# Tongji-MIC-Lab/TDVC

Hardware: AMD Instinct MI355X
Metric: 1080p P-frames/sec (encode + reconstruct, lambda=2048 config) (higher is better)
Workload: dtype f16; 1 GPU; 1x 1920x1080 (padded 1088x1920) 7-frame synthetic GOP (seed 1234), batch 1, P-frames coded in GOP order; gop=7, batch=1, parallelism=gop-sharded x1, weights=closed-form filler (no checkpoint ships)

## Files before the change

tdvc_amd/csrc/conv_mfma.hip:

```cpp
#include "conv_common.h"

using convk::ConvParams;

namespace {

constexpr int TH = 8, TW = 32;

template <int CK8, int MT, int STRIDE, bool LEAN = false>
__global__ __launch_bounds__(256, LEAN ? 3 : 1) void conv_mfma_kernel(const ConvParams p) {
  extern __shared__ __attribute__((aligned(16))) unsigned char smem[];
  constexpr int CK = CK8 * 8;
  constexpr int PS = (CK8 == 1) ? 16 : CK * 2 + 16;
  int* tapoff = reinterpret_cast<int*>(smem);
  unsigned char* tile = smem + 256;

  const int tid = threadIdx.x, lane = tid & 63, wave = tid >> 6;
  const int hh = lane >> 5, r = lane & 31;
  const int tile_id = p.reverse ? (int)gridDim.x - 1 - tdvc_xcd_tile(blockIdx.x) : tdvc_xcd_tile(blockIdx.x);
  const int tx = tile_id % p.tiles_x, ty = tile_id / p.tiles_x;
  const int cb = blockIdx.y, n = blockIdx.z;

  const int TIH = (TH - 1) * STRIDE + p.kh;
  const int TIW = (TW - 1) * STRIDE + p.kw;
  const int HALFW = (TIW + 1) >> 1;
  const int TIWp = (STRIDE == 2) ? 2 * HALFW : TIW;

  if (tid < p.ntaps) {
    const int dy = p.tap_dy[tid], dx = p.tap_dx[tid];
    tapoff[tid] = (STRIDE == 2) ? (dy * TIWp + (dx & 1) * HALFW + (dx >> 1)) * PS : (dy * TIWp + dx) * PS;
  }

  int base[2];
#pragma unroll
  for (int nt = 0; nt < 2; ++nt) base[nt] = (((wave * 2 + nt) * STRIDE) * TIWp + r) * PS;

  f32x16 acc[MT][2];
#pragma unroll
  for (int mt = 0; mt < MT; ++mt)
#pragma unroll
    for (int nt = 0; nt < 2; ++nt)
#pragma unroll
      for (int i = 0; i < 16; ++i) acc[mt][nt][i] = 0.f;

  const half_t* xn = p.x + (long)n * p.x_sn;
  const int iy0 = ty * TH * STRIDE - p.pad, ix0 = tx * TW * STRIDE - p.pad;
  const int total = TIH * TIW * CK8;

  for (int ch = 0; ch < p.nchunks; ++ch) {
    if (ch > 0) __syncthreads();
    for (int idx = tid; idx < total; idx += 256) {
      const int c8 = idx % CK8;
      const int pix = idx / CK8;
      const int c = pix % TIW, rr = pix / TIW;
      const int iy = iy0 + rr, ix = ix0 + c;
      const int cg = ch * CK + c8 * 8;
      half8 v = {0, 0, 0, 0, 0, 0, 0, 0};
      if (iy >= 0 && iy < p.H && ix >= 0 && ix < p.W && cg < p.Cin)
        v = *reinterpret_cast<const half8*>(xn + ((long)iy * p.W + ix) * p.x_sp + cg);
      if (p.square) v = v * v;
      const int cpos = (STRIDE == 2) ? ((c & 1) * HALFW + (c >> 1)) : c;
      *reinterpret_cast<half8*>(tile + (rr * TIWp + cpos) * PS + c8 * 16) = v;
    }
    __syncthreads();

    const half_t* wp[MT];
#pragma unroll
    for (int mt = 0; mt < MT; ++mt)
      wp[mt] = p.w + ((((long)(cb * MT + mt) * p.nchunks + ch) * p.steps) * 64 + lane) * 8;

    if constexpr (CK8 == 1) {
      for (int s = 0; s < p.steps; ++s) {
        int tap = 2 * s + hh;
        tap = tap < p.ntaps ? tap : p.ntaps - 1;
        const int toff = tapoff[tap];
        half8 a[MT], b[2];
#pragma unroll
        for (int mt = 0; mt < MT; ++mt) { a[mt] = *reinterpret_cast<const half8*>(wp[mt]); wp[mt] += 512; }
#pragma unroll
        for (int nt = 0; nt < 2; ++nt) b[nt] = *reinterpret_cast<const half8*>(tile + base[nt] + toff);
#pragma unroll
        for (int mt = 0; mt < MT; ++mt)
#pragma unroll
          for (int nt = 0; nt < 2; ++nt)
            acc[mt][nt] = __builtin_amdgcn_mfma_f32_32x32x16_f16(a[mt], b[nt], acc[mt][nt], 0, 0, 0);
      }
    } else {
      for (int tap = 0; tap < p.ntaps; ++tap) {
        const int toff = tapoff[tap] + hh * 16;
#pragma unroll
        for (int s2 = 0; s2 < CK8 / 2; ++s2) {
          half8 a[MT], b[2];
#pragma unroll
          for (int mt = 0; mt < MT; ++mt) { a[mt] = *reinterpret_cast<const half8*>(wp[mt]); wp[mt] += 512; }
#pragma unroll
          for (int nt = 0; nt < 2; ++nt)
            b[nt] = *reinterpret_cast<const half8*>(tile + base[nt] + toff + s2 * 32);
#pragma unroll
          for (int mt = 0; mt < MT; ++mt)
#pragma unroll
            for (int nt = 0; nt < 2; ++nt)
              acc[mt][nt] = __builtin_amdgcn_mfma_f32_32x32x16_f16(a[mt], b[nt], acc[mt][nt], 0, 0, 0);
        }
      }
    }
  }

  if constexpr (MT == 2 && LEAN) {
    __syncthreads();
    convk::epilogue_simple_rows<2, false, 2>(p, acc, p.bias + cb * 64, tile + wave * (32 * 144), n, cb * 64,
                                             ty * TH + wave * 2, tx * TW, lane, false);
    return;
  } else if constexpr (MT == 2) {
    if (p.simple) {
      __syncthreads();
      convk::epilogue_simple_rows<2, false, 1>(p, acc, p.bias + cb * 64, tile + wave * (32 * 144), n, cb * 64,
                                               ty * TH + wave * 2, tx * TW, lane, false);
      return;
    }
  }
  const int ox = tx * TW + r;
#pragma unroll
  for (int nt = 0; nt < 2; ++nt) {
    const int oy = ty * TH + wave * 2 + nt;
    if (oy >= p.Ho || ox >= p.Wo) continue;
#pragma unroll
    for (int mt = 0; mt < MT; ++mt) {
#pragma unroll
      for (int g = 0; g < 4; ++g) {
        const int co = (cb * MT + mt) * 32 + 8 * g + 4 * hh;
        float v[4];
#pragma unroll
        for (int i = 0; i < 4; ++i) v[i] = acc[mt][nt][4 * g + i];
        convk::epilogue4(p, n, oy, ox, co, v);
      }
    }
  }
}

template <int CK8, int MT, int STRIDE>
int launch(const ConvParams& p, dim3 grid, size_t lds, hipStream_t st) {
  if constexpr (MT == 2) {
    if (p.simple == 2) {
      hipLaunchKernelGGL((conv_mfma_kernel<CK8, MT, STRIDE, true>), grid, dim3(256), lds, st, p);
      return tdvc_launch_status("tdvc_conv2d");
    }
  }
  hipLaunchKernelGGL((conv_mfma_kernel<CK8, MT, STRIDE, false>), grid, dim3(256), lds, st, p);
  return tdvc_launch_status("tdvc_conv2d");
}

template <int CK8, int MT>
int launch_s(const ConvParams& p, int stride, dim3 grid, size_t lds, hipStream_t st) {
  return stride == 1 ? launch<CK8, MT, 1>(p, grid, lds, st) : launch<CK8, MT, 2>(p, grid, lds, st);
}

template <int CK8>
int launch_m(const ConvParams& p, int mt, int stride, dim3 grid, size_t lds, hipStream_t st) {
  return mt == 1 ? launch_s<CK8, 1>(p, stride, grid, lds, st) : launch_s<CK8, 2>(p, stride, grid, lds, st);
}

inline int lds_bytes(int ck, int kh, int kw, int stride) {
  const int ps = (ck == 8) ? 16 : ck * 2 + 16;
  const int tih = (TH - 1) * stride + kh, tiw = (TW - 1) * stride + kw;
  const int tiwp = stride == 2 ? 2 * ((tiw + 1) >> 1) : tiw;
  return 256 + tih * tiwp * ps;
}

inline int cout_tiles(int cout) { return cout <= 32 ? 1 : 2 * ((cout + 63) / 64); }

}

extern "C" int tdvc_conv_plan(int cin, int kh, int kw, int stride) {
  if (cin <= 0 || (cin % 8) != 0 || kh < 1 || kw < 1 || kh > 7 || kw > 7 || (stride != 1 && stride != 2)) {
    tdvc_set_error("tdvc_conv_plan: unsupported geometry cin=%d k=%dx%d stride=%d", cin, kh, kw, stride);
    return TDVC_EINVAL;
  }
  const int cands[4] = {64, 32, 16, 8};
  for (int i = 0; i < 4; ++i) {
    const int ck = cands[i];
    if (ck > cin && ck != 8) {
      if (cin % ck != 0 && cin < ck) continue;
    }
    if (lds_bytes(ck, kh, kw, stride) <= 64 * 1024) return ck;
  }
  tdvc_set_error("tdvc_conv_plan: no LDS plan for k=%dx%d stride=%d", kh, kw, stride);
  return TDVC_EINVAL;
}

extern "C" int64_t tdvc_conv_packed_bytes(int cout, int cin, int ntaps, int ck) {
  if (cout <= 0 || cin <= 0 || ntaps <= 0 || ntaps > TDVC_MAX_TAPS || (ck != 8 && ck != 16 && ck != 32 && ck != 64)) return TDVC_EINVAL;
  const int ck8 = ck / 8;
  const int64_t nchunks = (cin + ck - 1) / ck;
  const int64_t steps = (ntaps * ck8 + 1) / 2;
  return (int64_t)cout_tiles(cout) * nchunks * steps * 64 * 8 * 2;
}

extern "C" int tdvc_pack_conv_weights(const float* w, int cout, int cin_real, int cin, int kh, int kw,
                                      int ntaps, const int8_t* tap_dy, const int8_t* tap_dx, int ck, uint16_t* dst) {
  TDVC_CHECK(w && dst && tap_dy && tap_dx, "tdvc_pack_conv_weights: null pointer");
  TDVC_CHECK(tdvc_conv_packed_bytes(cout, cin, ntaps, ck) > 0, "tdvc_pack_conv_weights: bad geometry");
  TDVC_CHECK(cin_real <= cin, "tdvc_pack_conv_weights: cin_real > cin");
  const int ck8 = ck / 8;
  const int nchunks = (cin + ck - 1) / ck;
  const int steps = (ntaps * ck8 + 1) / 2;
  const int tiles = cout_tiles(cout);
  half_t* out = reinterpret_cast<half_t*>(dst);
  for (int t = 0; t < tiles; ++t)
    for (int ch = 0; ch < nchunks; ++ch)
      for (int s = 0; s < steps; ++s)
        for (int lane = 0; lane < 64; ++lane) {
          const int r = lane & 31, h = lane >> 5;
          const int co = t * 32 + r;
          const int kc = 2 * s + h;
          half_t* o = out + ((((int64_t)t * nchunks + ch) * steps + s) * 64 + lane) * 8;
          for (int j = 0; j < 8; ++j) {
            float v = 0.f;
            if (kc < ntaps * ck8 && co < cout) {
              const int tap = kc / ck8, c8 = kc % ck8;
              const int ci = ch * ck + c8 * 8 + j;
              const int dy = tap_dy[tap], dx = tap_dx[tap];
              if (ci < cin_real && dy >= 0 && dy < kh && dx >= 0 && dx < kw)
                v = w[(((int64_t)co * cin_real + ci) * kh + dy) * kw + dx];
            }
            o[j] = (half_t)v;
          }
        }
  return TDVC_OK;
}

int conv_direct_lds_bytes(const tdvc_conv_desc* d) { return lds_bytes(d->ck, d->kh, d->kw, d->stride); }
int conv_cout_tiles(int cout) { return cout_tiles(cout); }

int launch_conv_direct(const ConvParams& p, int ck8, int stride, int N, hipStream_t st) {
  const int tiles = cout_tiles(p.cout), mt = tiles == 1 ? 1 : 2;
  const int lds = lds_bytes(ck8 * 8, p.kh, p.kw, stride);
  const dim3 grid(p.tiles_x * ((p.Ho + TH - 1) / TH), tiles / mt, N);
  const size_t lds_v1 = (p.simple && lds < 256 + 4 * 32 * 144) ? 256 + 4 * 32 * 144 : lds;
  switch (ck8) {
    case 1: return launch_m<1>(p, mt, stride, grid, lds_v1, st);
    case 2: return launch_m<2>(p, mt, stride, grid, lds_v1, st);
    case 4: return launch_m<4>(p, mt, stride, grid, lds_v1, st);
    default: return launch_m<8>(p, mt, stride, grid, lds_v1, st);
  }
}
```

tdvc_amd/csrc/conv_n16.hip:

```cpp
#include "conv_common.h"

using convk::ConvParams;

namespace {

constexpr int N16_TH = 8, N16_TW = 64, N16_NTHR = 512;

struct N16Extra {
  int ksteps;
  int ps;
  int a_bytes;
  int ntiles, tiles_x;
  int cin_shift;
};

template <int NCB>
__global__ __launch_bounds__(N16_NTHR, 1) void conv_n16_kernel(const ConvParams p, const N16Extra e) {
  extern __shared__ __attribute__((aligned(16))) unsigned char smem[];
  unsigned char* wl = smem;
  unsigned char* tile = wl + e.a_bytes;
  const int tid = threadIdx.x, lane = tid & 63;
  const int wave = __builtin_amdgcn_readfirstlane(tid >> 6);
  const int px = lane & 15, kg = lane >> 4;
  const int TIW = N16_TW + p.kw - 1, TIH = N16_TH + p.kh - 1;
  const int cin = p.Cin, c8n = cin >> 3;

  for (int i = tid; i < e.ksteps * NCB * 64; i += N16_NTHR) {
    const int ln = i & 63, cb = (i >> 6) % NCB, S = (i >> 6) / NCB;
    const int q = 4 * S + (ln >> 4), s = q >> 1, h = q & 1;
    half8 v = {0, 0, 0, 0, 0, 0, 0, 0};
    if (s < p.steps) v = *reinterpret_cast<const half8*>(p.w + ((long)s * 64 + (16 * cb + (ln & 15)) + 32 * h) * 8);
    *reinterpret_cast<half8*>(wl + (long)i * 16) = v;
  }

  const int base = (wave * TIW + px) * e.ps;
  const int cstep = 16 * e.ps;
  auto frag_off = [&](int S) {
    const int kk0 = 32 * S + 8 * kg;
    const int tap = min(kk0 >> e.cin_shift, p.ntaps - 1);
    const int dy = tap / p.kw, dx = tap - dy * p.kw;
    return base + (dy * TIW + dx) * e.ps + (kk0 & (cin - 1)) * 2;
  };

  for (int tile_i = blockIdx.x; tile_i < e.ntiles; tile_i += gridDim.x) {
    const int per_img = e.tiles_x * ((p.Ho + N16_TH - 1) / N16_TH);
    const int n = tile_i / per_img, rem = tile_i - n * per_img;
    const int ty = rem / e.tiles_x, tx = rem - ty * e.tiles_x;
    const half_t* xn = p.x + (long)n * p.x_sn;
    const int iy0 = ty * N16_TH - p.pad, ix0 = tx * N16_TW - p.pad;
    __syncthreads();
    const int total = TIH * TIW * c8n;
    for (int idx0 = tid; idx0 < total; idx0 += 8 * N16_NTHR) {
      half8 v[8];
#pragma unroll
      for (int u = 0; u < 8; ++u) {
        const int idx = idx0 + u * N16_NTHR;
        const int pix = idx >> (e.cin_shift - 3), c8 = idx & (c8n - 1);
        const int rr = pix / TIW, cc = pix - rr * TIW;
        const int iy = iy0 + rr, ix = ix0 + cc;
        const bool ok = (int)(idx < total) & (int)(iy >= 0) & (int)(iy < p.H) & (int)(ix >= 0) & (int)(ix < p.W);
        const half_t* src = xn + ((long)(ok ? iy : 0) * p.W + (ok ? ix : 0)) * p.x_sp + c8 * 8;
        typedef unsigned u32x4 __attribute__((ext_vector_type(4)));
        u32x4 bits = *reinterpret_cast<const u32x4*>(src);
        unsigned m = ok ? 0xFFFFFFFFu : 0u;
        asm volatile("" : "+v"(m));
        bits &= m;
        v[u] = __builtin_bit_cast(half8, bits);
      }
#pragma unroll
      for (int u = 0; u < 8; ++u) {
        const int idx = idx0 + u * N16_NTHR;
        if (idx < total) {
          const int pix = idx >> (e.cin_shift - 3), c8 = idx & (c8n - 1);
          *reinterpret_cast<half8*>(tile + pix * e.ps + c8 * 16) = v[u];
        }
      }
    }
    __syncthreads();

    f32x4 acc[NCB][4];
#pragma unroll
    for (int cb = 0; cb < NCB; ++cb)
#pragma unroll
      for (int c = 0; c < 4; ++c) acc[cb][c] = f32x4{0.f, 0.f, 0.f, 0.f};

    half8 a0[NCB], b0[4], a1[NCB], b1[4];
    auto load = [&](int S, half8 (&a)[NCB], half8 (&b)[4]) {
      const int off = frag_off(S);
#pragma unroll
      for (int cb = 0; cb < NCB; ++cb) a[cb] = *reinterpret_cast<const half8*>(wl + ((S * NCB + cb) * 64 + lane) * 16);
#pragma unroll
      for (int c = 0; c < 4; ++c) b[c] = *reinterpret_cast<const half8*>(tile + off + c * cstep);
    };
    auto mm = [&](half8 (&a)[NCB], half8 (&b)[4]) {
#pragma unroll
      for (int c = 0; c < 4; ++c)
#pragma unroll
        for (int cb = 0; cb < NCB; ++cb) acc[cb][c] = __builtin_amdgcn_mfma_f32_16x16x32_f16(a[cb], b[c], acc[cb][c], 0, 0, 0);
    };
    const int KS = e.ksteps;
    load(0, a0, b0);
    for (int S = 0; S < KS; S += 2) {
      load(min(S + 1, KS - 1), a1, b1);
      mm(a0, b0);
      load(min(S + 2, KS - 1), a0, b0);
      if (S + 1 < KS) mm(a1, b1);
    }

    const int oy = ty * N16_TH + wave;
#pragma unroll
    for (int c = 0; c < 4; ++c) {
      const int ox = tx * N16_TW + 16 * c + px;
      if (oy < p.Ho && ox < p.Wo) {
#pragma unroll
        for (int cb = 0; cb < NCB; ++cb) {
          float v[4] = {acc[cb][c][0], acc[cb][c][1], acc[cb][c][2], acc[cb][c][3]};
          convk::epilogue4(p, n, oy, ox, 16 * cb + 4 * kg, v);
        }
      }
    }
  }
}

inline int n16_ps(int cin) { return 2 * cin + 16; }
inline int n16_ksteps(int ntaps, int cin) { return (ntaps * cin + 31) / 32; }
inline int n16_lds(int cin, int kh, int kw, int ntaps, int ncb) {
  return n16_ksteps(ntaps, cin) * ncb * 1024 + (N16_TH + kh - 1) * (N16_TW + kw - 1) * n16_ps(cin);
}

}

bool conv_n16_eligible(const tdvc_conv_desc* d, int Ho, int Wo) {
  const int cin = d->x.C;
  const bool cin_ok = cin == 8 || cin == 16 || cin == 32 || cin == 64;
  const bool dense = convk::taps_dense(d, d->kh, d->kw, d->pad);
  return cin_ok && dense && d->ck == cin && d->stride == 1 && d->cout <= 32 && !d->s2d && !d->square_input && !d->gdn &&
         (long)Ho * Wo >= convk::LARGE_MAP_PIXELS &&
         n16_lds(cin, d->kh, d->kw, d->ntaps, d->cout <= 16 ? 1 : 2) <= 150 * 1024;
}

int launch_conv_n16(const ConvParams& p, int N, hipStream_t st) {
  const int ncb = p.cout <= 16 ? 1 : 2;
  N16Extra e;
  e.ksteps = n16_ksteps(p.ntaps, p.Cin);
  e.ps = n16_ps(p.Cin);
  e.a_bytes = e.ksteps * ncb * 1024;
  e.tiles_x = (p.Wo + N16_TW - 1) / N16_TW;
  e.ntiles = N * e.tiles_x * ((p.Ho + N16_TH - 1) / N16_TH);
  e.cin_shift = p.Cin == 8 ? 3 : p.Cin == 16 ? 4 : p.Cin == 32 ? 5 : 6;
  const int lds = n16_lds(p.Cin, p.kh, p.kw, p.ntaps, ncb);
  const int per_cu = lds <= 78 * 1024 ? 2 : 1;
  int grid = e.ntiles < 256 * per_cu ? e.ntiles : 256 * per_cu;
  const auto go = ncb == 1 ? convk::launch_big_lds<&conv_n16_kernel<1>, ConvParams, N16Extra> : convk::launch_big_lds<&conv_n16_kernel<2>, ConvParams, N16Extra>;
  return go("tdvc_conv2d(n16)", 160 * 1024, dim3(grid), dim3(N16_NTHR), lds, st, p, e);
}
```

Before: 47.65 frames/s.

## Add wide-tile MFMA conv kernel and prefetch pipeline for n16 conv

Adds a new direct-conv kernel for single-cout-tile stride-1 layers on large maps. It uses 16-row tiles with 32x32x16 MFMAs over four row tiles per wave and a double-buffered LDS ring for weights. Separately, the n16 kernel gains a register prefetch of the next tile's input, overlapping global loads with MFMA compute, plus a precomputed LDS table of k-step offsets and a three-stage fragment pipeline. Both are on by default through debug toggles, at the cost of more registers, more LDS, and more template variants.

```diff
diff --git a/tdvc_amd/csrc/conv_mfma.hip b/tdvc_amd/csrc/conv_mfma.hip
--- a/tdvc_amd/csrc/conv_mfma.hip
+++ b/tdvc_amd/csrc/conv_mfma.hip
@@ -135,6 +135,132 @@
       }
     }
   }
+}
+
+constexpr int WTH = 16, WGROUP = 4096;
+
+template <int CK8>
+__global__ __launch_bounds__(256, 2) void conv_mfma_wide_kernel(const ConvParams p) {
+  extern __shared__ __attribute__((aligned(16))) unsigned char smem[];
+  constexpr int CK = CK8 * 8, PS = CK * 2 + 16, K2 = CK8 / 2, NT = 4;
+  int* tapoff = reinterpret_cast<int*>(smem);
+  unsigned char* wring = smem + 256;
+  unsigned char* tile = smem + 256 + 2 * WGROUP;
+
+  const int tid = threadIdx.x, lane = tid & 63;
+  const int wave = __builtin_amdgcn_readfirstlane(tid >> 6);
+  const int hh = lane >> 5, r = lane & 31;
+  const int tile_id = p.reverse ? (int)gridDim.x - 1 - tdvc_xcd_tile(blockIdx.x) : tdvc_xcd_tile(blockIdx.x);
+  const int tx = tile_id % p.tiles_x, ty = tile_id / p.tiles_x;
+  const int n = blockIdx.z;
+  const int TIW = TW + p.kw - 1, TIH = WTH + p.kh - 1;
+  const int total = TIH * TIW * CK8;
+  const int ntaps = p.ntaps;
+
+  if (tid < ntaps) tapoff[tid] = (p.tap_dy[tid] * TIW + p.tap_dx[tid]) * PS;
+
+  const int F = p.nchunks * p.steps;
+  const half_t* wthread = p.w + lane * 8;
+  auto wsrc = [&](int g) -> const half_t* {
+    const int fr = min(4 * g + wave, F - 1);
+    return wthread + (long)fr * 512;
+  };
+  *reinterpret_cast<half8*>(wring + tid * 16) = *reinterpret_cast<const half8*>(wsrc(0));
+  half8 wreg = *reinterpret_cast<const half8*>(wsrc(1));
+
+  int base[NT];
+#pragma unroll
+  for (int nt = 0; nt < NT; ++nt) base[nt] = ((wave * NT + nt) * TIW + r) * PS + hh * 16;
+
+  f32x16 acc[NT];
+#pragma unroll
+  for (int nt = 0; nt < NT; ++nt)
+#pragma unroll
+    for (int i = 0; i < 16; ++i) acc[nt][i] = 0.f;
+
+  const half_t* xn = p.x + (long)n * p.x_sn;
+  const int iy0 = ty * WTH - p.pad, ix0 = tx * TW - p.pad;
+
+  int f = 0;
+  for (int ch = 0; ch < p.nchunks; ++ch) {
+    if (ch > 0) __syncthreads();
+    for (int idx0 = tid; idx0 < total; idx0 += 8 * 256) {
+      half8 v[8];
+#pragma unroll
+      for (int u = 0; u < 8; ++u) {
+        const int idx = idx0 + u * 256;
+        const int c8 = idx & (CK8 - 1), pix = idx / CK8;
+        const int rr = pix / TIW, c = pix - rr * TIW;
+        const int iy = iy0 + rr, ix = ix0 + c;
+        const int cg = ch * CK + c8 * 8;
+        const bool ok = (int)(idx < total) & (int)(iy >= 0) & (int)(iy < p.H) & (int)(ix >= 0) & (int)(ix < p.W) & (int)(cg < p.Cin);
+        const half_t* src = xn + ((long)(ok ? iy : 0) * p.W + (ok ? ix : 0)) * p.x_sp + (ok ? cg : 0);
+        typedef unsigned u32x4 __attribute__((ext_vector_type(4)));
+        u32x4 bits = *reinterpret_cast<const u32x4*>(src);
+        unsigned m = ok ? 0xFFFFFFFFu : 0u;
+        asm volatile("" : "+v"(m));
+        bits &= m;
+        v[u] = __builtin_bit_cast(half8, bits);
+      }
+#pragma unroll
+      for (int u = 0; u < 8; ++u) {
+        const int idx = idx0 + u * 256;
+        if (idx < total) {
+          if (p.square) v[u] = v[u] * v[u];
+          *reinterpret_cast<half8*>(tile + (idx / CK8) * PS + (idx & (CK8 - 1)) * 16) = v[u];
+        }
+      }
+    }
+    __syncthreads();
+
+    for (int tap = 0; tap < ntaps; ++tap) {
+      if ((f & 3) == 0) {
+        const int g = f >> 2;
+        *reinterpret_cast<half8*>(wring + ((g + 1) & 1) * WGROUP + tid * 16) = wreg;
+        wreg = *reinterpret_cast<const half8*>(wsrc(g + 2));
+      }
+      const unsigned char* wslot = wring + ((f >> 2) & 1) * WGROUP + (f & 3) * 1024 + lane * 16;
+      const int toff = tapoff[tap];
+#pragma unroll
+      for (int s2 = 0; s2 < K2; ++s2) {
+        half8 b[NT];
+        const half8 a = *reinterpret_cast<const half8*>(wslot + s2 * 1024);
+#pragma unroll
+        for (int nt = 0; nt < NT; ++nt) b[nt] = *reinterpret_cast<const half8*>(tile + base[nt] + toff + s2 * 32);
+#pragma unroll
+        for (int nt = 0; nt < NT; ++nt) acc[nt] = __builtin_amdgcn_mfma_f32_32x32x16_f16(a, b[nt], acc[nt], 0, 0, 0);
+      }
+      f += K2;
+      if ((f & 3) == 0) __syncthreads();
+    }
+  }
+
+  const int ox = tx * TW + r;
+#pragma unroll
+  for (int nt = 0; nt < NT; ++nt) {
+    const int oy = ty * WTH + wave * NT + nt;
+    if (oy >= p.Ho || ox >= p.Wo) continue;
+#pragma unroll
+    for (int g = 0; g < 4; ++g) {
+      float v[4];
+#pragma unroll
+      for (int i = 0; i < 4; ++i) v[i] = acc[nt][4 * g + i];
+      convk::epilogue4(p, n, oy, ox, 8 * g + 4 * hh, v);
+    }
+  }
+}
+
+inline int wide_lds_bytes(int ck, int kh, int kw) { return 256 + 2 * WGROUP + (WTH + kh - 1) * (TW + kw - 1) * (ck * 2 + 16); }
+
+constexpr int WIDE_LDS_LIMIT = 160 * 1024;
+
+int g_direct_form = 1;
+
+inline bool wide_form_takes(const ConvParams& p, int ck8, int mt, int stride, int N) {
+  if (!(mt == 1 && stride == 1 && (ck8 == 2 || ck8 == 4 || ck8 == 8) && (long)N * p.Ho * p.Wo >= convk::LARGE_MAP_PIXELS &&
+        wide_lds_bytes(ck8 * 8, p.kh, p.kw) <= WIDE_LDS_LIMIT))
+    return false;
+  return g_direct_form == 2 || (long)N * p.tiles_x * ((p.Ho + WTH - 1) / WTH) >= 512;
 }
 
 template <int CK8, int MT, int STRIDE>
@@ -231,9 +357,18 @@
 int conv_direct_lds_bytes(const tdvc_conv_desc* d) { return lds_bytes(d->ck, d->kh, d->kw, d->stride); }
 int conv_cout_tiles(int cout) { return cout_tiles(cout); }
 
+extern "C" void tdvc_debug_set_direct_form(int form) { g_direct_form = form; }
+
 int launch_conv_direct(const ConvParams& p, int ck8, int stride, int N, hipStream_t st) {
   const int tiles = cout_tiles(p.cout), mt = tiles == 1 ? 1 : 2;
   const int lds = lds_bytes(ck8 * 8, p.kh, p.kw, stride);
+  if (g_direct_form && wide_form_takes(p, ck8, mt, stride, N)) {
+    const dim3 wgrid(p.tiles_x * ((p.Ho + WTH - 1) / WTH), 1, N);
+    const auto go = ck8 == 2   ? convk::launch_big_lds<&conv_mfma_wide_kernel<2>, ConvParams>
+                    : ck8 == 4 ? convk::launch_big_lds<&conv_mfma_wide_kernel<4>, ConvParams>
+                               : convk::launch_big_lds<&conv_mfma_wide_kernel<8>, ConvParams>;
+    return go("tdvc_conv2d", WIDE_LDS_LIMIT, wgrid, dim3(256), wide_lds_bytes(ck8 * 8, p.kh, p.kw), st, p);
+  }
   const dim3 grid(p.tiles_x * ((p.Ho + TH - 1) / TH), tiles / mt, N);
   const size_t lds_v1 = (p.simple && lds < 256 + 4 * 32 * 144) ? 256 + 4 * 32 * 144 : lds;
   switch (ck8) {
diff --git a/tdvc_amd/csrc/conv_n16.hip b/tdvc_amd/csrc/conv_n16.hip
--- a/tdvc_amd/csrc/conv_n16.hip
+++ b/tdvc_amd/csrc/conv_n16.hip
@@ -14,7 +14,7 @@
   int cin_shift;
 };
 
-template <int NCB>
+template <int NCB, int PF>
 __global__ __launch_bounds__(N16_NTHR, 1) void conv_n16_kernel(const ConvParams p, const N16Extra e) {
   extern __shared__ __attribute__((aligned(16))) unsigned char smem[];
   unsigned char* wl = smem;
@@ -24,6 +24,49 @@
   const int px = lane & 15, kg = lane >> 4;
   const int TIW = N16_TW + p.kw - 1, TIH = N16_TH + p.kh - 1;
   const int cin = p.Cin, c8n = cin >> 3;
+  typedef unsigned u32x4 __attribute__((ext_vector_type(4)));
+
+  const int per_img = e.tiles_x * ((p.Ho + N16_TH - 1) / N16_TH);
+  const int total = TIH * TIW * c8n;
+  u32x4 pf[PF > 0 ? PF : 1];
+  unsigned pf_ok = 0;
+  auto prefetch = [&](int tile_i) {
+    const int n = tile_i / per_img, rem = tile_i - n * per_img;
+    const int ty = rem / e.tiles_x, tx = rem - ty * e.tiles_x;
+    const half_t* xn = p.x + (long)n * p.x_sn;
+    const int iy0 = ty * N16_TH - p.pad, ix0 = tx * N16_TW - p.pad;
+    pf_ok = 0;
+    int t = tid;
+    asm volatile("" : "+v"(t));
+#pragma unroll
+    for (int u = 0; u < PF; ++u) {
+      const int idx = t + u * N16_NTHR;
+      const int pix = idx >> (e.cin_shift - 3), c8 = idx & (c8n - 1);
+      const int rr = pix / TIW, cc = pix - rr * TIW;
+      const int iy = iy0 + rr, ix = ix0 + cc;
+      const bool ok = (int)(idx < total) & (int)(iy >= 0) & (int)(iy < p.H) & (int)(ix >= 0) & (int)(ix < p.W);
+      const half_t* src = xn + ((long)(ok ? iy : 0) * p.W + (ok ? ix : 0)) * p.x_sp + c8 * 8;
+      pf[u] = *reinterpret_cast<const u32x4*>(src);
+      pf_ok |= (ok ? 1u : 0u) << u;
+    }
+  };
+  auto commit = [&]() {
+    int t = tid;
+    asm volatile("" : "+v"(t));
+#pragma unroll
+    for (int u = 0; u < PF; ++u) {
+      const int idx = t + u * N16_NTHR;
+      if (idx < total) {
+        const int pix = idx >> (e.cin_shift - 3), c8 = idx & (c8n - 1);
+        unsigned m = 0u - ((pf_ok >> u) & 1u);
+        asm volatile("" : "+v"(m));
+        *reinterpret_cast<u32x4*>(tile + pix * e.ps + c8 * 16) = pf[u] & m;
+      }
+    }
+  };
+  if constexpr (PF > 0) {
+    if ((int)blockIdx.x < e.ntiles) prefetch(blockIdx.x);
+  }
 
   for (int i = tid; i < e.ksteps * NCB * 64; i += N16_NTHR) {
     const int ln = i & 63, cb = (i >> 6) % NCB, S = (i >> 6) / NCB;
@@ -42,41 +85,54 @@
     return base + (dy * TIW + dx) * e.ps + (kk0 & (cin - 1)) * 2;
   };
 
+  int* koff = reinterpret_cast<int*>(tile + TIH * TIW * e.ps);
+  if constexpr (PF > 0) {
+    for (int i = tid; i < e.ksteps * 4; i += N16_NTHR) {
+      const int kk0 = 8 * i;
+      const int tap = min(kk0 >> e.cin_shift, p.ntaps - 1);
+      const int dy = tap / p.kw, dx = tap - dy * p.kw;
+      koff[i] = (dy * TIW + dx) * e.ps + (kk0 & (cin - 1)) * 2;
+    }
+  }
+
   for (int tile_i = blockIdx.x; tile_i < e.ntiles; tile_i += gridDim.x) {
-    const int per_img = e.tiles_x * ((p.Ho + N16_TH - 1) / N16_TH);
     const int n = tile_i / per_img, rem = tile_i - n * per_img;
     const int ty = rem / e.tiles_x, tx = rem - ty * e.tiles_x;
-    const half_t* xn = p.x + (long)n * p.x_sn;
-    const int iy0 = ty * N16_TH - p.pad, ix0 = tx * N16_TW - p.pad;
     __syncthreads();
-    const int total = TIH * TIW * c8n;
-    for (int idx0 = tid; idx0 < total; idx0 += 8 * N16_NTHR) {
-      half8 v[8];
-#pragma unroll
-      for (int u = 0; u < 8; ++u) {
-        const int idx = idx0 + u * N16_NTHR;
-        const int pix = idx >> (e.cin_shift - 3), c8 = idx & (c8n - 1);
-        const int rr = pix / TIW, cc = pix - rr * TIW;
-        const int iy = iy0 + rr, ix = ix0 + cc;
-        const bool ok = (int)(idx < total) & (int)(iy >= 0) & (int)(iy < p.H) & (int)(ix >= 0) & (int)(ix < p.W);
-        const half_t* src = xn + ((long)(ok ? iy : 0) * p.W + (ok ? ix : 0)) * p.x_sp + c8 * 8;
-        typedef unsigned u32x4 __attribute__((ext_vector_type(4)));
-        u32x4 bits = *reinterpret_cast<const u32x4*>(src);
-        unsigned m = ok ? 0xFFFFFFFFu : 0u;
-        asm volatile("" : "+v"(m));
-        bits &= m;
-        v[u] = __builtin_bit_cast(half8, bits);
-      }
-#pragma unroll
-      for (int u = 0; u < 8; ++u) {
-        const int idx = idx0 + u * N16_NTHR;
-        if (idx < total) {
+    if constexpr (PF > 0) {
+      commit();
+      __syncthreads();
+      prefetch(min(tile_i + (int)gridDim.x, e.ntiles - 1));
+    } else {
+      const half_t* xn = p.x + (long)n * p.x_sn;
+      const int iy0 = ty * N16_TH - p.pad, ix0 = tx * N16_TW - p.pad;
+      for (int idx0 = tid; idx0 < total; idx0 += 8 * N16_NTHR) {
+        half8 v[8];
+#pragma unroll
+        for (int u = 0; u < 8; ++u) {
+          const int idx = idx0 + u * N16_NTHR;
           const int pix = idx >> (e.cin_shift - 3), c8 = idx & (c8n - 1);
-          *reinterpret_cast<half8*>(tile + pix * e.ps + c8 * 16) = v[u];
-        }
-      }
-    }
-    __syncthreads();
+          const int rr = pix / TIW, cc = pix - rr * TIW;
+          const int iy = iy0 + rr, ix = ix0 + cc;
+          const bool ok = (int)(idx < total) & (int)(iy >= 0) & (int)(iy < p.H) & (int)(ix >= 0) & (int)(ix < p.W);
+          const half_t* src = xn + ((long)(ok ? iy : 0) * p.W + (ok ? ix : 0)) * p.x_sp + c8 * 8;
+          u32x4 bits = *reinterpret_cast<const u32x4*>(src);
+          unsigned m = ok ? 0xFFFFFFFFu : 0u;
+          asm volatile("" : "+v"(m));
+          bits &= m;
+          v[u] = __builtin_bit_cast(half8, bits);
+        }
+#pragma unroll
+        for (int u = 0; u < 8; ++u) {
+          const int idx = idx0 + u * N16_NTHR;
+          if (idx < total) {
+            const int pix = idx >> (e.cin_shift - 3), c8 = idx & (c8n - 1);
+            *reinterpret_cast<half8*>(tile + pix * e.ps + c8 * 16) = v[u];
+          }
+        }
+      }
+      __syncthreads();
+    }
 
     f32x4 acc[NCB][4];
 #pragma unroll
@@ -100,11 +156,42 @@
     };
     const int KS = e.ksteps;
     load(0, a0, b0);
-    for (int S = 0; S < KS; S += 2) {
-      load(min(S + 1, KS - 1), a1, b1);
-      mm(a0, b0);
-      load(min(S + 2, KS - 1), a0, b0);
-      if (S + 1 < KS) mm(a1, b1);
+    if constexpr (PF > 0) {
+      half8 a2[NCB], b2[4];
+      auto ko = [&](int S) { return koff[4 * min(S, KS - 1) + kg]; };
+      auto load_at = [&](int S, int off, half8 (&a)[NCB], half8 (&b)[4]) {
+#pragma unroll
+        for (int cb = 0; cb < NCB; ++cb) a[cb] = *reinterpret_cast<const half8*>(wl + ((S * NCB + cb) * 64 + lane) * 16);
+#pragma unroll
+        for (int c = 0; c < 4; ++c) b[c] = *reinterpret_cast<const half8*>(tile + base + off + c * cstep);
+      };
+      load_at(min(1, KS - 1), ko(1), a1, b1);
+      int o_next = ko(2), o_after = ko(3);
+      for (int S = 0; S < KS; S += 3) {
+        load_at(min(S + 2, KS - 1), o_next, a2, b2);
+        o_next = o_after;
+        o_after = ko(S + 4);
+        mm(a0, b0);
+        if (S + 1 < KS) {
+          load_at(min(S + 3, KS - 1), o_next, a0, b0);
+          o_next = o_after;
+          o_after = ko(S + 5);
+          mm(a1, b1);
+        }
+        if (S + 2 < KS) {
+          load_at(min(S + 4, KS - 1), o_next, a1, b1);
+          o_next = o_after;
+          o_after = ko(S + 6);
+          mm(a2, b2);
+        }
+      }
+    } else {
+      for (int S = 0; S < KS; S += 2) {
+        load(min(S + 1, KS - 1), a1, b1);
+        mm(a0, b0);
+        load(min(S + 2, KS - 1), a0, b0);
+        if (S + 1 < KS) mm(a1, b1);
+      }
     }
 
     const int oy = ty * N16_TH + wave;
@@ -138,6 +225,23 @@
          (long)Ho * Wo >= convk::LARGE_MAP_PIXELS &&
          n16_lds(cin, d->kh, d->kw, d->ntaps, d->cout <= 16 ? 1 : 2) <= 150 * 1024;
 }
+
+namespace {
+int g_n16_form = 1;
+int g_n16_grid_cap = 0;
+
+int launch_n16(int ncb, int pf, const char* what, dim3 grid, int lds, hipStream_t st, const ConvParams& p, const N16Extra& e) {
+  const auto go = ncb == 2  ? convk::launch_big_lds<&conv_n16_kernel<2, 0>, ConvParams, N16Extra>
+                  : pf == 0 ? convk::launch_big_lds<&conv_n16_kernel<1, 0>, ConvParams, N16Extra>
+                  : pf == 4 ? convk::launch_big_lds<&conv_n16_kernel<1, 4>, ConvParams, N16Extra>
+                  : pf == 8 ? convk::launch_big_lds<&conv_n16_kernel<1, 8>, ConvParams, N16Extra>
+                            : convk::launch_big_lds<&conv_n16_kernel<1, 12>, ConvParams, N16Extra>;
+  return go(what, 160 * 1024, grid, dim3(N16_NTHR), lds, st, p, e);
+}
+}
+
+extern "C" void tdvc_debug_set_conv_n16_form(int form) { g_n16_form = form; }
+extern "C" void tdvc_debug_set_conv_n16_grid_cap(int cap) { g_n16_grid_cap = cap; }
 
 int launch_conv_n16(const ConvParams& p, int N, hipStream_t st) {
   const int ncb = p.cout <= 16 ? 1 : 2;
@@ -148,9 +252,12 @@
   e.tiles_x = (p.Wo + N16_TW - 1) / N16_TW;
   e.ntiles = N * e.tiles_x * ((p.Ho + N16_TH - 1) / N16_TH);
   e.cin_shift = p.Cin == 8 ? 3 : p.Cin == 16 ? 4 : p.Cin == 32 ? 5 : 6;
-  const int lds = n16_lds(p.Cin, p.kh, p.kw, p.ntaps, ncb);
+  int lds = n16_lds(p.Cin, p.kh, p.kw, p.ntaps, ncb);
+  const int loads = ((N16_TH + p.kh - 1) * (N16_TW + p.kw - 1) * (p.Cin >> 3) + N16_NTHR - 1) / N16_NTHR;
+  const int pf = !g_n16_form || ncb == 2 || loads > 12 ? 0 : loads <= 4 ? 4 : loads <= 8 ? 8 : 12;
   const int per_cu = lds <= 78 * 1024 ? 2 : 1;
+  if (pf) lds += e.ksteps * 16;
   int grid = e.ntiles < 256 * per_cu ? e.ntiles : 256 * per_cu;
-  const auto go = ncb == 1 ? convk::launch_big_lds<&conv_n16_kernel<1>, ConvParams, N16Extra> : convk::launch_big_lds<&conv_n16_kernel<2>, ConvParams, N16Extra>;
-  return go("tdvc_conv2d(n16)", 160 * 1024, dim3(grid), dim3(N16_NTHR), lds, st, p, e);
-}
+  if (g_n16_grid_cap > 0 && grid > g_n16_grid_cap) grid = g_n16_grid_cap;
+  return launch_n16(ncb, pf, "tdvc_conv2d(n16)", dim3(grid), lds, st, p, e);
+}
```

Result: no change. 48.13 frames/s (median of 6 runs) (+1.0%).
